# pvjosue/CWFA

Measured on AMD Instinct MI355X. Metric: volumes/sec inverse-pass @512×512×96 fp32; NLL match vs ref (1/2/4/8 GPU), higher is better.
Workload: dtype f32 (storage, accumulation, wavelets, couplings); convolution products on the bf16 matrix cores from an exact three-way bf16 split of both fp32 operands, six products per fp32 product: fp32-equivalent; plain-fp32-MFMA figure: fp32_mfma; 1 GPU; 512x512x96 volume, 4-scale CWFA (CAT blocks, 64 ch) + LRNN inverse, z=0, batch 1/GPU, random-init weights (BASELINE.json configs[2]); precision=split, parallelism=replicated x1 (independent volumes per GPU, no collective)

## Files before the change

### cwfa_amd/_lib.py

```python
import ctypes as C
import os

_HERE = os.path.dirname(os.path.abspath(__file__))
LIB_PATH = os.path.join(_HERE, "libcwfa_hip.so")

CLAMP = {"NONE": 0, "ATAN": 1, "TANH": 2, "SIGMOID": 3}
ACT = {None: 0, "none": 0, "elu": 1, "prelu": 2, "gelu": 3, "relu": 4}
CHAIN_MAX = 8

c_f32p = C.c_void_p
c_i64p = C.c_void_p
c_f64p = C.c_void_p


class AffineStage(C.Structure):
    _fields_ = [("s_raw", c_f32p), ("t", c_f32p), ("s_bs", C.c_int64), ("t_bs", C.c_int64), ("clamp_kind", C.c_int),
                ("clamp", C.c_float), ("pre_scale", C.c_float), ("t_neg_div_sqrt2", C.c_int), ("perm", c_i64p),
                ("perm_axis", C.c_int), ("gin", C.c_int)]


class Chain(C.Structure):
    _fields_ = [("n_stages", C.c_int), ("stage", AffineStage * CHAIN_MAX), ("src_c", C.c_void_p), ("src_h", C.c_void_p)]


class ChainGrads(C.Structure):
    _fields_ = [("ds", c_f32p * CHAIN_MAX), ("dt", c_f32p * CHAIN_MAX), ("ds_bs", C.c_int64 * CHAIN_MAX),
                ("dt_bs", C.c_int64 * CHAIN_MAX)]


class ConvOpts(C.Structure):
    _fields_ = [("bias", c_f32p), ("act", C.c_int), ("prelu_alpha", c_f32p), ("residual", c_f32p), ("res_bs", C.c_int64),
                ("act2", C.c_int), ("in_scale", c_f32p), ("in_shift", c_f32p), ("in_affine_bs", C.c_int), ("in_add", c_f32p),
                ("in_add_bs", C.c_int64), ("upshuffle2", C.c_int), ("in_blocked8", C.c_int), ("out_blocked8", C.c_int),
                ("in_cat", c_f32p), ("in_cat_bs", C.c_int64), ("in_cat_from", C.c_int), ("in_cat_c1", C.c_int), ("out_stats", c_f64p), ("prelu_per_channel", C.c_int)]


class Couple(C.Structure):
    _fields_ = [("x", c_f32p), ("y", c_f32p), ("x_bs", C.c_int64), ("y_bs", C.c_int64), ("n", C.c_int), ("clamp_kind", C.c_int),
                ("clamp", C.c_float), ("pre_scale", C.c_float), ("rev", C.c_int), ("logdet", c_f64p), ("in_blocked8", C.c_int)]


class EvalAffine(C.Structure):
    _fields_ = [("enabled", C.c_int), ("scale", C.c_float), ("std", C.c_float), ("mean", C.c_float)]


class EvalPost(C.Structure):
    _fields_ = [("normalize", C.c_int), ("threshold", C.c_int), ("norm_sub", C.c_float), ("norm_div", C.c_float),
                ("vol_min", C.c_float), ("lower", C.c_float), ("upper", C.c_float), ("clamp_value", C.c_float)]

# ... 12 lines not shown
    "cwfa_set_option": (i, [C.c_char_p, i]),
    "cwfa_haar1d_fwd_f32": (i, [p, p, p, i, i, i64, i64, i64, i64, p]),
    "cwfa_haar1d_inv_f32": (i, [p, p, p, i, i, i64, i64, i64, i64, p]),
    "cwfa_haar2d_fwd_f32": (i, [p, p, i, i, i, i, i, f, p]),
    "cwfa_haar2d_inv_f32": (i, [p, p, i, i, i, i, i, f, p]),
    "cwfa_haar3d_fwd_f32": (i, [p, p, i, i, i, i, i, f, i64, p]),
    "cwfa_haar3d_inv_f32": (i, [p, p, i, i, i, i, i, f, i64, p]),
    "cwfa_gather_f32": (i, [p, p, p, i, i, i, i, i, i64, i64, p]),
    "cwfa_affine_f32": (i, [p, p, C.POINTER(AffineStage), i, i, i, i, i, i64, i64, p, p, p]),
    "cwfa_channel_affine_f32": (i, [p, p, p, p, i, p, p, i, i, i64, i64, i64, p]),
    "cwfa_chain_inv_f32": (i, [p, p, p, C.POINTER(Chain), i, i, i, i, i64, i64, i64, p, p]),
    "cwfa_chain_fwd_f32": (i, [p, p, p, C.POINTER(Chain), p, i, i, i, i, i64, i64, i64, p, p, p]),
    "cwfa_conv2d_packed_floats": (i64, [i, i, i]),
    "cwfa_conv2d_pack_f32": (i, [p, p, i, i, i, i, p]),
    "cwfa_conv2d_f32": (i, [p, p, p, i, i, i, i, i, i, i64, i64, C.POINTER(ConvOpts), p]),
    "cwfa_subnet_pack1x1_f32": (i, [p, p, p]),
    "cwfa_subnet_layer_tape_f32": (i, [p, p, p, p, p, p, p, i, i, i, i64, i64, i64, p]),
    "cwfa_subnet_layer_f32": (i, [p, p, p, p, p, p, i, i, i, i64, i64, p]),
    "cwfa_conv3d_1k1_f32": (i, [p, p, p, p, p, p, p, i, i, i, i, i, p]),
    "cwfa_conv3d_1k1_split_f32": (i, [p, p, p, p, p, p, p, i, i, i, i, i, p]),
    "cwfa_channel_stats_f32": (i, [p, p, i, i, i64, i64, p]),
    "cwfa_bn_fold_f32": (i, [p, d, p, p, p, p, f, p, i, p, p, i, p]),
    "cwfa_maxpool_f32": (i, [p, p, p, p, p, i, i, i, i, i, i, p]),
    "cwfa_sample_stats_f32": (i, [p, p, i, i64, p]),
    "cwfa_layernorm_apply_f32": (i, [p, p, p, p, f, p, i, i64, p]),
    "cwfa_attention_combine_f32": (i, [p, p, p, p, p, p, p, p, i, i, i64, p]),
    "cwfa_scale_channels_f32": (i, [p, p, p, i, i, i64, p]),
    "cwfa_axpby_f32": (i, [p, p, f, f, p, i64, p]),
    "cwfa_bn_running_update_f32": (i, [p, C.c_double, f, p, p, p, i, p]),
    "cwfa_bn_finish_f32": (i, [p, d, p, p, p, f, i, p, p, f, p, p, f, f, i, p, p, i, i, p]),
# ... 87 lines not shown
```

### cwfa_amd/csrc/conv2d.hip

```cpp
#include "conv_internal.h"

#include <string.h>
#include <type_traits>

namespace {

template <int KS_, int CK_, int MT_, int NT_, int WM_, int WN_, int XV_ = 1>
struct Cfg {
    static constexpr int KS = KS_, CK = CK_, MT = MT_, NT = NT_, WM = WM_, WN = WN_;
    static constexpr int XV = XV_;
    static_assert(XV_ == 1 || (XV_ == 4 && KS_ == 1), "vector staging needs halo-free tiles");
    static constexpr int PAD = KS / 2;
    static constexpr int NTHREADS = 64 * WM * WN;
    static constexpr int CT = 32 * MT * WM;
    static constexpr int TR = NT * WN;
    static constexpr int TC = 32;
    static constexpr int XR = TR + KS - 1;
    static constexpr int XC = TC + KS - 1;
    static constexpr int XS = CK * XR * XC;
    static constexpr int XS_PAD = (XS + 3) & ~3;
    static constexpr int WS = KS * KS * CK * CT;
    static constexpr int XPT = (XS / XV + NTHREADS - 1) / NTHREADS;
    static constexpr int WPT = (WS / 4 + NTHREADS - 1) / NTHREADS;
    static constexpr int BUF = XS_PAD + WS;
// ... 557 lines not shown
namespace {

int fill_params(ConvParams& p, const char* name, const float* x, const float* w_packed, float* y, int B, int Cin, int H,
                int W, int Cout, int64_t x_bs, int64_t y_bs, const cwfa_conv_opts* opts) {
    CWFA_REQUIRE(B >= 0 && Cin > 0 && Cout > 0 && H >= 0 && W >= 0, CWFA_E_INVAL, "%s: bad size", name);
    if (B == 0 || H == 0 || W == 0) return 1;
    CWFA_REQUIRE(x && w_packed && y, CWFA_E_INVAL, "%s: null pointer", name);
    CWFA_REQUIRE((int64_t)Cin * H * W < (1ll << 30) && (int64_t)Cout * H * W * (p.o.upshuffle2 ? 1 : 1) < (1ll << 30), CWFA_E_SHAPE, "%s: C*H*W exceeds the 32-bit byte offsets of a tile (2^30 elements per image)", name);
    CWFA_REQUIRE(cwfa_aligned16(w_packed), CWFA_E_ALIGN, "%s: packed weights must be 16-byte aligned", name);
    p.x = x; p.wp = w_packed; p.y = y;
    p.B = B; p.Cin = Cin; p.H = H; p.W = W; p.Cout = Cout;
    p.x_bs = x_bs; p.y_bs = y_bs;
    p.products = g_cwfa_operand == CwfaOperand::split3 ? 6 : 1;
    if (opts) p.o = *opts;
    CWFA_REQUIRE(!(p.o.in_scale && !p.o.in_shift), CWFA_E_INVAL, "%s: in_scale without in_shift", name);
    CWFA_REQUIRE(p.o.act >= 0 && p.o.act <= CWFA_ACT_RELU && p.o.act2 >= 0 && p.o.act2 <= CWFA_ACT_RELU, CWFA_E_INVAL,
                 "%s: bad activation", name);
    CWFA_REQUIRE(!((p.o.act == CWFA_ACT_PRELU || p.o.act2 == CWFA_ACT_PRELU) && !p.o.prelu_alpha), CWFA_E_INVAL,
                 "%s: PReLU without prelu_alpha", name);
    return CWFA_OK;
}

typedef Cfg<1, 16, 2, 4, 4, 2> CS;
constexpr int CS_XB = 3 * 2 * 8 * 32 * 16, CS_WB = 3 * 2 * 256 * 16, CS_BUFB = CS_XB + CS_WB;

__device__ __forceinline__ void split3(float v, unsigned short (&o)[3]) {
    const __bf16 a1 = (__bf16)v;
    const float r1 = v - (float)a1;
    const __bf16 a2 = (__bf16)r1;
    const float r2 = r1 - (float)a2;
// ... 390 lines not shown
            default: return launch<C1v_128, N | U | K, U>(p, epi, st);
        }
    }
    switch (s.id) {
        case 0: return launch<C3_32, N | P | RP, 0>(p, epi, st);
        case 1: return launch<C3_64, N | E | P | RP, 0>(p, epi, st);
        case 2: return launch<C3_128, N | P, P>(p, epi, st);
        case 3: return launch<C1_32, N | P | G, P>(p, epi, st);
        case 4: return launch<C1_64, N | RE | G | K, 0>(p, epi, st);
        case 5: return launch<C1_128, N | U | K, U>(p, epi, st);
        case 6: return launch<C7_32, N, 0>(p, epi, st);
        default: return launch<C7_64, N, 0>(p, epi, st);
    }
}

extern "C" int cwfa_subnet_pack1x1_f32(const float* w, float* panel, void* stream) {
    CWFA_REQUIRE(w && panel, CWFA_E_INVAL, "cwfa_subnet_pack1x1_f32: null pointer");
    hipLaunchKernelGGL(pack1x1_kernel, dim3(16), dim3(256), 0, (hipStream_t)stream, w, panel);
    CWFA_LAUNCH_CHECK("cwfa_subnet_pack1x1_f32");
    return CWFA_OK;
}

extern "C" int cwfa_subnet_layer_tape_f32(const float* x, const float* w3_packed, const float* b3, const float* w1_panel,
                                          const float* b1, float* y, float* hidden, int B, int H, int W, int64_t x_bs, int64_t y_bs,
                                          int64_t hidden_bs, void* stream) {
    ConvParams p{};
    cwfa_conv_opts o{};
    o.bias = b3;
    int rc = fill_params(p, "cwfa_subnet_layer_tape_f32", x, w3_packed, y, B, 64, H, W, 64, x_bs, y_bs, &o);
    if (rc) return rc < 0 ? rc : CWFA_OK;
// ... 31 lines not shown
```

### cwfa_amd/csrc/conv_split3x3.hip

```cpp
#include "conv_internal.h"

extern int g_cwfa_split_xcd_map;
extern int g_cwfa_split_rows16;

namespace {

constexpr int TR = 8, TC = 32;

template <int KS, int RPW = 4>
struct XG {
    static constexpr int TRW = 2 * RPW, NT = 2 * RPW;
    static constexpr int PAD = KS / 2, XR = TRW + 2 * PAD, XC = TC + 2 * PAD, NTAP = KS * KS;
    static constexpr int EPK = XR * XC;
    static constexpr int KHB = KS == 7 ? 8512 : RPW == 8 ? 9792 : 5440;
    static constexpr int XPB = 2 * KHB;
    static constexpr int XB = 3 * XPB;
    static constexpr bool SPECIAL = KS == 3 && RPW == 4;
    static constexpr int NEK = SPECIAL ? 2 : 3;
    static_assert(EPK * 16 <= KHB && KHB % 256 == 64 && 2 * EPK <= 512 * NEK, "staging entry map");
    static_assert(!SPECIAL || (EPK > 256 && EPK <= 384), "3x3 staging entry map");
    static_assert(KS == 3 || RPW == 4, "7x7: 8-row tiles");
};

template <int MPW, int KS = 3, int RPW = 4, int WM = 4>
// ... 67 lines not shown
            ekh[k] = e >= EPK;
            eidx[k] = e - ekh[k] * EPK;
            fin[k] = e < 2 * EPK;
        }
    }
    bool fok[NEK];
#pragma unroll
    for (int k = 0; k < NEK; ++k) {
        const int r = eidx[k] / XC, c = eidx[k] % XC;
        const int gr = row0 + r - PAD, gc = col0 + c - PAD;
        fok[k] = fin[k] && gr >= 0 && gr < p.H && gc >= 0 && gc < p.W;
        fo[k] = !fok[k] ? OOB : p.o.in_blocked8 ? (unsigned)((gr * p.W + gc) * 32) : (unsigned)((gr * p.W + gc) * 4);
        if constexpr (!SPECIAL) fo[k] = !fok[k] ? OOB : fo[k] + (unsigned)(ekh[k] * 8) * (unsigned)plane;
    }
    const int xbytes = p.Cin * plane;
    const auto rx = CWFA_RSRC(p.x + (int64_t)b * p.x_bs, xbytes);
    const auto ra = CWFA_RSRC(ADD ? p.o.in_add + (int64_t)b * p.o.in_add_bs : p.x, ADD ? xbytes : 0);
    const bool has_aff = p.o.in_scale != nullptr;
    typedef const float __attribute__((address_space(4))) cfloat;
    cfloat* sc = has_aff ? (cfloat*)(p.o.in_scale + (int64_t)b * p.o.in_affine_bs) : nullptr;
    cfloat* sh = has_aff ? (cfloat*)(p.o.in_shift + (int64_t)b * p.o.in_affine_bs) : nullptr;

    auto load_entry = [&](auto kc, float (&xv)[8], float (&av)[8], int chunk) {
        constexpr int k = decltype(kc)::value;
        const int ch0 = chunk * 16 + (SPECIAL ? ekh[k] * 8 : 0);
        if (KS == 3 && !ADD && p.o.in_blocked8) {
            const f32x4 lo4 = __builtin_bit_cast(f32x4, __builtin_amdgcn_raw_buffer_load_b128(rx, fo[k], ch0 * plane, 0));
            const f32x4 hi4 = __builtin_bit_cast(f32x4, __builtin_amdgcn_raw_buffer_load_b128(rx, fo[k], ch0 * plane + 16, 0));
#pragma unroll
            for (int j = 0; j < 4; ++j) {
                xv[j] = lo4[j];
                xv[4 + j] = hi4[j];
// ... 515 lines not shown
    CWFA_REQUIRE(B >= 0 && Cin > 0 && Cout > 0 && H >= 0 && W >= 0, CWFA_E_INVAL, "cwfa_conv3x3_split_f32: bad size");
    if (B == 0 || H == 0 || W == 0) return CWFA_OK;
    CWFA_REQUIRE(x && w_packed && y, CWFA_E_INVAL, "cwfa_conv3x3_split_f32: null pointer");
    CWFA_REQUIRE(cwfa_aligned16(w_packed), CWFA_E_ALIGN, "cwfa_conv3x3_split_f32: packed weights must be 16-byte aligned");
    SParams p{};
    p.x = x; p.wp = w_packed; p.y = y;
    p.B = B; p.Cin = Cin; p.H = H; p.W = W; p.Cout = Cout; p.x_bs = x_bs; p.y_bs = y_bs;
    if (opts) p.o = *opts;
    CWFA_REQUIRE(!p.o.upshuffle2 && !p.o.in_cat, CWFA_E_SHAPE, "cwfa_conv3x3_split_f32: upshuffle2 / in_cat are 1x1 features");
    CWFA_REQUIRE(!p.o.in_blocked8 || (Cin % 8 == 0 && cwfa_aligned16(x) && (x_bs & 3) == 0 && !p.o.in_add), CWFA_E_ALIGN,
                 "cwfa_conv3x3_split_f32: blocked input needs Cin %% 8 == 0, 16-byte alignment and no added tensor");
    CWFA_REQUIRE(!p.o.out_blocked8 || (Cout % 8 == 0 && cwfa_aligned16(y) && (y_bs & 3) == 0 && !p.o.residual && p.o.act2 == CWFA_ACT_NONE &&
                                       (p.o.act == CWFA_ACT_NONE || p.o.act == CWFA_ACT_PRELU)),
                 CWFA_E_ALIGN, "cwfa_conv3x3_split_f32: blocked output needs Cout %% 8 == 0, 16-byte alignment and a bias / PReLU epilogue");
    CWFA_REQUIRE(!(p.o.in_scale && !p.o.in_shift), CWFA_E_INVAL, "cwfa_conv3x3_split_f32: in_scale without in_shift");
    CWFA_REQUIRE(!p.o.out_stats || (!p.o.out_blocked8 && !p.o.residual && p.o.act2 == CWFA_ACT_NONE &&
                                    (p.o.act == CWFA_ACT_NONE || p.o.act == CWFA_ACT_PRELU)),
                 CWFA_E_INVAL, "cwfa_conv3x3_split_f32: out_stats needs an NCHW output and a bias / PReLU epilogue");
    CWFA_REQUIRE(!((p.o.out_stats || p.o.out_blocked8) && p.o.in_add && p.o.act == CWFA_ACT_NONE), CWFA_E_INVAL,
                 "cwfa_conv3x3_split_f32: out_stats / out_blocked8 with in_add need a PReLU epilogue");
    CWFA_REQUIRE(p.o.act >= 0 && p.o.act <= CWFA_ACT_RELU && p.o.act2 >= 0 && p.o.act2 <= CWFA_ACT_RELU, CWFA_E_INVAL,
                 "cwfa_conv3x3_split_f32: bad activation");
    CWFA_REQUIRE(!((p.o.act == CWFA_ACT_PRELU || p.o.act2 == CWFA_ACT_PRELU) && !p.o.prelu_alpha), CWFA_E_INVAL,
                 "cwfa_conv3x3_split_f32: PReLU without prelu_alpha");
    p.nchunks = (Cin + 15) / 16;
    p.nsteps = nsteps_of(Cin);
    p.nrun = p.nsteps - ((p.nchunks & 1) ? 4 : 0);
    p.tiles_x = (W + TC - 1) / TC;
    const int mpw = mpw_of(Cout);
    CWFA_REQUIRE((int64_t)(Cin + 64) * H * W * 4 < (1ll << 31) && (int64_t)(Cout + 64 * mpw) * H * W * 4 < (1ll << 31) &&
// ... 40 lines not shown
    pack_bank(w, packed, Cout, Cin, 64, 49, (hipStream_t)stream);
    CWFA_LAUNCH_CHECK("cwfa_conv7x7_split_pack_f32");
    return CWFA_OK;
}

extern "C" int cwfa_conv7x7_split_f32(const float* x, const void* w_packed, float* y, int B, int Cin, int H, int W, int Cout,
                                      int64_t x_bs, int64_t y_bs, const cwfa_conv_opts* opts, void* stream) {
    CWFA_REQUIRE(B >= 0 && Cin > 0 && Cout > 0 && Cout <= 64 && H >= 0 && W >= 0, CWFA_E_INVAL, "cwfa_conv7x7_split_f32: bad size (Cout <= 64)");
    if (B == 0 || H == 0 || W == 0) return CWFA_OK;
    CWFA_REQUIRE(x && w_packed && y, CWFA_E_INVAL, "cwfa_conv7x7_split_f32: null pointer");
    CWFA_REQUIRE(cwfa_aligned16(w_packed), CWFA_E_ALIGN, "cwfa_conv7x7_split_f32: packed weights must be 16-byte aligned");
    SParams p{};
    p.x = x; p.wp = w_packed; p.y = y;
    p.B = B; p.Cin = Cin; p.H = H; p.W = W; p.Cout = Cout; p.x_bs = x_bs; p.y_bs = y_bs;
    if (opts) p.o = *opts;
    CWFA_REQUIRE(!p.o.upshuffle2 && !p.o.in_cat && !p.o.in_scale && !p.o.in_add && !p.o.in_blocked8 && !p.o.out_blocked8 && !p.o.residual && !p.o.out_stats &&
                     p.o.act == CWFA_ACT_NONE && p.o.act2 == CWFA_ACT_NONE,
                 CWFA_E_INVAL, "cwfa_conv7x7_split_f32: bias-only epilogue, no load-side prologue, NCHW maps");
    p.nchunks = (Cin + 15) / 16;
    p.nsteps = nsteps_of(Cin, 49);
    p.nrun = p.nsteps;
    p.tiles_x = (W + TC - 1) / TC;
    CWFA_REQUIRE((int64_t)(Cin + 64) * H * W * 4 < (1ll << 31) && (int64_t)(Cout + 64) * H * W * 4 < (1ll << 31), CWFA_E_SHAPE,
                 "cwfa_conv7x7_split_f32: one sample's input / output must stay below 2 GiB");
    CWFA_REQUIRE((int64_t)p.tiles_x * ((H + TR - 1) / TR) < (1ll << 31) && B <= 65535, CWFA_E_SHAPE, "cwfa_conv7x7_split_f32: grid too large");
    hipStream_t st = (hipStream_t)stream;
    return launch<2, false, CWFA_ACT_NONE, 7, 4, 2>(p, st);
}
```

### cwfa_amd/ops.py

```python
import ctypes as C

import torch

from . import _lib
from ._lib import AffineStage, Chain, ConvOpts, check

__all__ = ["haar1d", "haar2d", "gather", "affine", "channel_affine", "chain_inv", "chain_fwd", "pack_conv_weight",
           "conv2d", "conv2d_wgrad", "elu_bwd", "set_precision", "gelu_add", "gelu_bwd", "layernorm_bwd", "attention_bwd", "plane_affine", "bn_bwd_stats", "bn_act_bwd", "maxpool2_bwd", "chain_bwd", "chain_inv_bwd", "prelu_bwd", "conv3d_1k1_backward", "pack_1x1_panel", "pack_split_layer_weight", "subnet_layer", "conv3d_1k1", "channel_stats", "bn_fold", "bn_running_update", "maxpool", "sample_stats", "layernorm_apply",
           "attention_combine", "scale_channels", "axpby", "stage"]


def _stream():
    return C.c_void_p(torch.cuda.current_stream().cuda_stream)


def _p(t):
    return None if t is None else C.c_void_p(t.data_ptr())


def _dev(t, name="tensor"):
    if not torch.is_tensor(t):
        raise TypeError(f"{name}: expected a torch.Tensor, got {type(t)}")
    if not t.is_cuda:
        raise RuntimeError(f"{name}: cwfa_amd runs on MI355X only -- got a {t.device} tensor (no CPU fallback exists)")
# ... 361 lines not shown
    start = (c1 + 15) // 16 * 16
    wz = torch.zeros((cout, start + cin - c1, 1, 1), dtype=torch.float32, device=w.device)
    wz[:, :c1] = w[:, :c1]
    wz[:, start:] = w[:, c1:]
    pc = pack_conv_weight(wz)
    pc.version, pc.src_ptr = w._version, w.data_ptr()
    pc.cat_c1, pc.cat_from = c1, start
    return pc


def conv_writes_stats(pc, act=None, residual=None, act2=None, out_blocked=False, in_add=False):
    return bool(pc.split and pc.ks == 3 and act in (None, "prelu") and residual is None and act2 is None and not out_blocked
                and not (in_add and act is None))


def conv2d(x, pc, bias=None, act=None, prelu_alpha=None, residual=None, act2=None, in_scale=None, in_shift=None,
           in_add=None, out=None, in_blocked=False, out_blocked=False, cat=None, out_stats=None):
    L = _lib.lib()
    x, xbs = planes(x, "x")
    B, Cin, H, W = x.shape
    o = ConvOpts()
    keep = [x]
    if cat is not None:
        cat, cbs = planes(cat, "cat")
        c1 = getattr(pc, "cat_c1", None)
        if c1 is None or Cin != c1 or tuple(cat.shape) != (B, pc.cin - pc.cat_from, H, W) or in_scale is not None or in_add is not None:
            raise ValueError("conv2d: `cat` needs a bank from pack_conv_weight_cat for exactly these two inputs, and no load-side prologue")
        o.in_cat, o.in_cat_bs, o.in_cat_from, o.in_cat_c1 = cat.data_ptr(), cbs, pc.cat_from, c1
        keep.append(cat)
        Cin = pc.cin
    if Cin != pc.cin:
        raise ValueError(f"conv2d: input has {Cin} channels, filter bank expects {pc.cin}")
# ... 26 lines not shown
            raise ValueError(f"conv2d: residual {tuple(residual.shape)} != output {oshape}")
        o.residual, o.res_bs = residual.data_ptr(), rbs
        keep.append(residual)
    if in_scale is not None:
        o.in_scale, o.in_shift = _dev(in_scale).data_ptr(), _dev(in_shift).data_ptr()
        if in_scale.numel() not in (Cin, B * Cin) or in_shift.numel() != in_scale.numel():
            raise ValueError("conv2d: in_scale / in_shift must be [Cin] or [B,Cin]")
        o.in_affine_bs = Cin if (in_scale.numel() == B * Cin and B > 1) else 0
    if in_add is not None:
        in_add, abs_ = planes(in_add, "in_add")
        if tuple(in_add.shape) != tuple(x.shape):
            raise ValueError("conv2d: in_add shape mismatch")
        o.in_add, o.in_add_bs = in_add.data_ptr(), abs_
        keep.append(in_add)
    o.upshuffle2 = int(up)
    if in_blocked:
        if not (pc.split and pc.ks == 3):
            raise ValueError("conv2d: channel-blocked input is read by the split-bf16 3x3 kernel only")
        o.in_blocked8 = 1
    if out_blocked:
        ok3 = (pc.split and pc.ks == 3 and pc.cout % 8 == 0 and residual is None and act2 is None and act in (None, "prelu")
               and not split3x3_narrow(pc.cout) and not (in_add is not None and act is None))
        ok1 = not pc.split and pc.ks == 1 and pc.cout >= 33 and pc.cout % 8 == 0 and not up
        if not (ok3 or ok1):
            raise ValueError("conv2d: channel-blocked output is written by the split-bf16 3x3 kernel (bias / PReLU) and by the "
                             "direct 1x1 kernel with 40..64 output channels only")
        o.out_blocked8 = 1
    if out_stats is not None:
        if not conv_writes_stats(pc, act, residual, act2, out_blocked, in_add is not None):
            raise ValueError("conv2d: out_stats needs the split-bf16 3x3 kernel with an NCHW output and a bias / PReLU epilogue")
# ... 27 lines not shown
                                       for i in range(B)], 0)
                if in_add is not None:
                    x = axpby(x.contiguous(), 1.0, in_add, 1.0)
            x, xbs = planes(x, "x")
            o.in_scale = o.in_shift = o.in_add = None
        check(L.cwfa_conv3x3_split_f32(_p(x), _p(pc.packed), _p(out), B, Cin, H, W, pc.cout, xbs, ybs, C.byref(o),
                                       _stream()), "conv3x3_split")
    elif pc.split:
        ws = torch.empty(L.cwfa_split_workspace_bytes(B, Cin, H * W), dtype=torch.uint8, device=x.device)
        per_sample = in_scale is not None and in_scale.numel() == B * Cin and B > 1
        check(L.cwfa_split_input_f32(_p(x), _p(ws), B, Cin, H * W, xbs, _p(in_scale), _p(in_shift), Cin if per_sample else 0,
                                     _p(in_add), in_add.stride(0) if in_add is not None else 0, _stream()), "split_input")
        o.in_scale = o.in_shift = o.in_add = None
        check(L.cwfa_conv_split_f32(_p(ws), _p(pc.packed), _p(out), B, Cin, H, W, pc.cout, pc.ks, ybs, C.byref(o), _stream()),
              "conv_split")
    else:
        check(L.cwfa_conv2d_f32(_p(x), _p(pc.packed), _p(out), B, Cin, H, W, pc.cout, pc.ks, xbs, ybs, C.byref(o),
                                _stream()), "conv2d")
    if rec is not None and rec.want(key):
        e1.record()
        rec.add(key, e0, e1)
    return out


def pack_couple_weight(w, bias):
    L = _lib.lib()
    w = _dev(w, "weight").detach()
    n2, cin, ks, kw = w.shape
    if ks != 3 or kw != 3 or n2 % 2 or n2 // 2 > 64:
        raise ValueError(f"pack_couple_weight: a [2n,Cin,3,3] bank with n <= 64 is needed, got {tuple(w.shape)}")
# ... 923 lines not shown
```

### cwfa_amd/unet.py

```python
import torch
from torch import nn

from . import ops
from .amp import amp_entry

__all__ = ["UNet", "UNetConvBlock", "UNetUpBlock"]


_MATERIALIZE_UP = False
_MATERIALIZE = True


class _Packed:

    def __init__(self):
        self._c = {}

    def get(self, conv, transposed=False):
        w = conv.weight
        pc = self._c.get(id(conv))
        if pc is None or pc.version != w._version or pc.src_ptr != w.data_ptr() or pc.epoch != ops.pack_epoch():
            pc = self._c[id(conv)] = ops.pack_conv_weight(w, transposed=transposed)
        return pc


class _Drop:
    __slots__ = ("u", "p")

    def __init__(self, u, p):
        self.u, self.p = u, p

    def mask(self):
        return ((self.u >= self.p).to(torch.float32) / (1.0 - self.p)).contiguous()


STATS_IN_EPILOGUE = True


def _bn_batch_stats(bn):
    return bn.training or not bn.track_running_stats


def _bn_stats_buffer(bn, device):
    key = (str(device), torch.cuda.current_stream(device).cuda_stream)
    bufs = bn.__dict__.setdefault("_cwfa_stats", {})
    st = bufs.get(key)
    if st is None or getattr(bn, "_cwfa_stats_dirty", False):
        st = bufs[key] = torch.zeros(2 * bn.num_features, dtype=torch.float64, device=device)
    bn._cwfa_stats_dirty = True
    return st

# ... 72 lines not shown
        step = 3 if self.batch_norm else 2
        return [(mods[i], mods[i + 1], mods[i + 2] if self.batch_norm else None) for i in (0, step)]

    @staticmethod
    def _act(a):
        if isinstance(a, nn.PReLU):
            if a.weight.numel() != 1:
                raise NotImplementedError("per-channel PReLU")
            return "prelu", a.weight
        if isinstance(a, nn.ELU):
            return "elu", None
        if isinstance(a, nn.ReLU):
            return "relu", None
        raise NotImplementedError(f"activation {type(a).__name__} has no HIP epilogue")

    def run(self, x, in_affine=None, in_add=None, out_mask=None):
        aff = in_affine
        layers = self._layers()
        packs = [self._packed.get(conv) for conv, _, _ in layers]
        for li, (conv, act, bn) in enumerate(layers):
            kind, alpha = self._act(act)
            sc, sh = aff if aff is not None else (None, None)
            add = in_add if li == 0 else None
            if (_MATERIALIZE and ops._split_bf16 < 2 and (sc is not None or add is not None)
                    and (x.shape[2] * x.shape[3]) % 4 == 0):
                x = ops.plane_affine(x, sc, sh, add=add)
                sc = sh = add = None
            st = None
            if (STATS_IN_EPILOGUE and bn is not None and _bn_batch_stats(bn)
                    and ops.conv_writes_stats(packs[li], kind, in_add=add is not None)):
                st = _bn_stats_buffer(bn, x.device)
            x = ops.conv2d(x, packs[li], bias=conv.bias, act=kind, prelu_alpha=alpha, in_scale=sc,
                           in_shift=sh, in_add=add, out_stats=st)
            last = li == len(layers) - 1
            m = out_mask if last else None
            if bn is not None:
                aff = _bn_affine(bn, x, m, stats=st)
            elif m is not None:
                aff = _drop_affine(x.shape[1], m)
            else:
                aff = None
        return x, aff

    @amp_entry
    def forward(self, x):
        y, aff = self.run(x)
        if aff is None:
            return y
# ... 7 lines not shown
        super().__init__()
        self.skip_conn = skip_conn
        if up_mode != 'upconv':
            raise NotImplementedError("cwfa_amd UNetUpBlock: up_mode='upconv' only (what the LRNN uses, networks.py:532)")
        self.up = nn.ConvTranspose2d(in_size, out_size, kernel_size=2, stride=2, bias=use_bias)
        in_size = out_size if not skip_conn else in_size // 2
        self.conv_block = UNetConvBlock(in_size, out_size, padding, batch_norm, use_bias=use_bias, activation=activation)
        self._packed = _Packed()

    @staticmethod
    def center_crop(layer, target_size):
        _, _, h, w = layer.size()
        dy, dx = (h - target_size[0]) // 2, (w - target_size[1]) // 2
        return layer[:, :, dy:(dy + target_size[0]), dx:(dx + target_size[1])]

    def run(self, x, bridge, in_affine=None, out_mask=None):
        sc, sh = in_affine if in_affine is not None else (None, None)
        if _MATERIALIZE_UP and ops._split_bf16 < 1 and sc is not None and (x.shape[2] * x.shape[3]) % 4 == 0:
            x = ops.plane_affine(x, sc, sh)
            sc = sh = None
        up = ops.conv2d(x, self._packed.get(self.up, transposed=True), bias=self.up.bias, in_scale=sc, in_shift=sh)
        add = self.center_crop(bridge, up.shape[2:]) if self.skip_conn else None
        return self.conv_block.run(up, in_add=add, out_mask=out_mask)

    @amp_entry
    def forward(self, x, bridge):
        y, aff = self.run(x, bridge)
        return y if aff is None else ops.channel_affine(y, aff[0], aff[1])


class UNet(nn.Module):

    def __init__(self, in_channels=1, n_classes=2, depth=5, wf=6, padding=True, batch_norm=True, up_mode='upsample',
                 drop_out=0, use_bias=False, skip_conn=False, activation=nn.PReLU):
        super().__init__()
        assert up_mode in ('upconv', 'upsample')
        self.padding, self.depth, self.skip_conn, self.drop_out = padding, depth, skip_conn, drop_out
        prev = in_channels
# ... 13 lines not shown
    @amp_entry
    def forward(self, x, store_activations=False, in_affine=None):
        if store_activations:
            raise NotImplementedError("store_activations is a debugging aid of the reference, not on the hot path")
        B, dev = x.shape[0], x.device
        skips, aff = [], in_affine
        n_draw = 0
        if self.drop_out:
            n_draw = B * (sum(d.block[0].out_channels for d in list(self.down_path)[:-1]) +
                          sum(u.conv_block.block[0].out_channels for u in self.up_path))
        pool = _DrawPool(n_draw, dev)
        for i, down in enumerate(self.down_path):
            x, aff = down.run(x, in_affine=aff)
            if i != len(self.down_path) - 1:
                sc, sh = aff if aff is not None else (None, None)
                x, full = ops.maxpool(x, x.shape[-1] // 2, x.shape[-1] // 2, sc, sh, want_full=True)
                skips.append(full)
                m = _drop(self.drop_out, B, x.shape[1], dev, pool)
                aff = _drop_affine(x.shape[1], m) if m is not None else None
        for i, up in enumerate(self.up_path):
            m = _drop(self.drop_out, B, up.conv_block.block[0].out_channels, dev, pool)
            x, aff = up.run(x, skips[-i - 1], in_affine=aff, out_mask=m)
        kind, alpha = UNetConvBlock._act(self.last[1])
        sc, sh = aff if aff is not None else (None, None)
        return ops.conv2d(x, self._packed.get(self.last[0]), bias=self.last[0].bias, act=kind, prelu_alpha=alpha,
                          in_scale=sc, in_shift=sh)
```

### include/cwfa_hip.h

```cpp
#ifndef CWFA_HIP_H
#define CWFA_HIP_H

#include <stdint.h>

#ifdef __cplusplus
extern "C" {
#endif

#define CWFA_VERSION 100

enum {
    CWFA_OK = 0,
    CWFA_E_INVAL = -1,
    CWFA_E_SHAPE = -2,
    CWFA_E_ALIGN = -3,
    CWFA_E_HIP = -4
};

enum { CWFA_CLAMP_NONE = 0, CWFA_CLAMP_ATAN = 1, CWFA_CLAMP_TANH = 2, CWFA_CLAMP_SIGMOID = 3 };

enum { CWFA_ACT_NONE = 0, CWFA_ACT_ELU = 1, CWFA_ACT_PRELU = 2, CWFA_ACT_GELU = 3, CWFA_ACT_RELU = 4 };

int cwfa_version(void);
const char* cwfa_last_error(void);
// ... 69 lines not shown
    int64_t res_bs;
    int act2;
    const float* in_scale;
    const float* in_shift;
    int in_affine_bs;
    const float* in_add;
    int64_t in_add_bs;
    int upshuffle2;
    int in_blocked8;
    int out_blocked8;
    const float* in_cat;
    int64_t in_cat_bs;
    int in_cat_from, in_cat_c1;
    double* out_stats;
    int prelu_per_channel;
} cwfa_conv_opts;

int cwfa_conv2d_f32(const float* x, const float* w_packed, float* y, int B, int Cin, int H, int W, int Cout, int ks,
                    int64_t x_bs, int64_t y_bs, const cwfa_conv_opts* opts, void* stream);

int cwfa_subnet_pack1x1_f32(const float* w, float* panel, void* stream);
int cwfa_subnet_layer_f32(const float* x, const float* w3_packed, const float* b3, const float* w1_panel, const float* b1,
                          float* y, int B, int H, int W, int64_t x_bs, int64_t y_bs, void* stream);
int cwfa_subnet_layer_tape_f32(const float* x, const float* w3_packed, const float* b3, const float* w1_panel, const float* b1,
                               float* y, float* hidden, int B, int H, int W, int64_t x_bs, int64_t y_bs, int64_t hidden_bs,
                               void* stream);

int cwfa_conv3d_1k1_f32(const float* x, const float* w1, const float* b1, const float* alpha, const float* w2,
                        const float* b2, float* y, int B, int D, int H, int W, int K, void* stream);
int cwfa_conv3d_1k1_split_f32(const float* x, const float* w1, const float* b1, const float* alpha, const float* w2,
                              const float* b2, float* y, int B, int D, int H, int W, int K, void* stream);


int cwfa_channel_stats_f32(const float* x, double* stats, int B, int C, int64_t HW, int64_t x_bs, void* stream);
// ... 161 lines not shown
```

Baseline: 53.95 volumes/s.

## Fuse skip-affine into up-path conv and add streaming narrow 1x1 conv kernel

Down-path skips are now kept raw (pre-BN-affine) together with their scale/shift. The first up-path split 3x3 conv applies that affine on the in_add operand, by swapping the roles of the x and add buffers. This avoids writing the full-resolution affined skip tensor during maxpool. A separate streaming kernel handles 1x1 convs with at most 8 outputs and 64 to 1024 inputs: it splits channels across four waves, keeps weights and the affine in LDS, and reduces partial sums in LDS. That kernel runs in plain fp32 FMA rather than the split path, and the fused-affine path is limited to certain output-bank widths.

After: 54.10 volumes/s (median of 6 runs). Within noise of the previous version (+0.3%).

```diff
diff --git a/cwfa_amd/_lib.py b/cwfa_amd/_lib.py
--- a/cwfa_amd/_lib.py
+++ b/cwfa_amd/_lib.py
@@ -32,7 +32,8 @@
     _fields_ = [("bias", c_f32p), ("act", C.c_int), ("prelu_alpha", c_f32p), ("residual", c_f32p), ("res_bs", C.c_int64),
                 ("act2", C.c_int), ("in_scale", c_f32p), ("in_shift", c_f32p), ("in_affine_bs", C.c_int), ("in_add", c_f32p),
                 ("in_add_bs", C.c_int64), ("upshuffle2", C.c_int), ("in_blocked8", C.c_int), ("out_blocked8", C.c_int),
-                ("in_cat", c_f32p), ("in_cat_bs", C.c_int64), ("in_cat_from", C.c_int), ("in_cat_c1", C.c_int), ("out_stats", c_f64p), ("prelu_per_channel", C.c_int)]
+                ("in_cat", c_f32p), ("in_cat_bs", C.c_int64), ("in_cat_from", C.c_int), ("in_cat_c1", C.c_int), ("out_stats", c_f64p), ("prelu_per_channel", C.c_int),
+                ("in_affine_on_add", C.c_int)]
 
 
 class Couple(C.Structure):
@@ -75,6 +76,7 @@
     "cwfa_conv2d_packed_floats": (i64, [i, i, i]),
     "cwfa_conv2d_pack_f32": (i, [p, p, i, i, i, i, p]),
     "cwfa_conv2d_f32": (i, [p, p, p, i, i, i, i, i, i, i64, i64, C.POINTER(ConvOpts), p]),
+    "cwfa_conv1x1_stream_f32": (i, [p, p, p, i, i, i64, i, i64, i64, C.POINTER(ConvOpts), p]),
     "cwfa_subnet_pack1x1_f32": (i, [p, p, p]),
     "cwfa_subnet_layer_tape_f32": (i, [p, p, p, p, p, p, p, i, i, i, i64, i64, i64, p]),
     "cwfa_subnet_layer_f32": (i, [p, p, p, p, p, p, i, i, i, i64, i64, p]),
diff --git a/cwfa_amd/csrc/conv2d.hip b/cwfa_amd/csrc/conv2d.hip
--- a/cwfa_amd/csrc/conv2d.hip
+++ b/cwfa_amd/csrc/conv2d.hip
@@ -595,6 +595,7 @@
     p.products = g_cwfa_operand == CwfaOperand::split3 ? 6 : 1;
     if (opts) p.o = *opts;
     CWFA_REQUIRE(!(p.o.in_scale && !p.o.in_shift), CWFA_E_INVAL, "%s: in_scale without in_shift", name);
+    CWFA_REQUIRE(!p.o.in_affine_on_add, CWFA_E_INVAL, "%s: in_affine_on_add is a cwfa_conv3x3_split_f32 feature", name);
     CWFA_REQUIRE(p.o.act >= 0 && p.o.act <= CWFA_ACT_RELU && p.o.act2 >= 0 && p.o.act2 <= CWFA_ACT_RELU, CWFA_E_INVAL,
                  "%s: bad activation", name);
     CWFA_REQUIRE(!((p.o.act == CWFA_ACT_PRELU || p.o.act2 == CWFA_ACT_PRELU) && !p.o.prelu_alpha), CWFA_E_INVAL,
@@ -1015,6 +1016,109 @@
     }
 }
 
+constexpr int S1_KG = 4, S1_ENT = 12, S1_MAXC = 1024;
+
+template <int CO>
+__global__ __launch_bounds__(64 * S1_KG) void conv1x1_stream_kernel(const float* __restrict__ x, const float* __restrict__ wp,
+                                                                    float* __restrict__ y, int Cin, int64_t HW, int64_t x_bs, int64_t y_bs,
+                                                                    cwfa_conv_opts o) {
+    extern __shared__ __attribute__((aligned(16))) float smem[];
+    const int tid = threadIdx.x, lane = tid & 63;
+    const int kg = __builtin_amdgcn_readfirstlane(tid >> 6);
+    const int b = blockIdx.y;
+    const bool aff = o.in_scale != nullptr;
+    for (int i = tid; i < Cin * S1_ENT; i += 64 * S1_KG) {
+        const int c = i / S1_ENT, j = i % S1_ENT;
+        float v = 0.f;
+        if (j < CO) v = wp[c * C1_32::CT + j];
+        else if (j == 8) v = aff ? o.in_scale[(int64_t)b * o.in_affine_bs + c] : 1.f;
+        else if (j == 9) v = aff ? o.in_shift[(int64_t)b * o.in_affine_bs + c] : 0.f;
+        smem[i] = v;
+    }
+    __syncthreads();
+    const int64_t q = (int64_t)blockIdx.x * 64 + lane, nq = HW >> 2;
+    const bool ok = q < nq;
+    const float* xp = x + (int64_t)b * x_bs + 4 * (ok ? q : 0);
+    const int cq = (Cin + S1_KG - 1) / S1_KG, c0 = kg * cq, c1 = c0 + cq < Cin ? c0 + cq : Cin;
+    f32x4 acc[CO];
+#pragma unroll
+    for (int k = 0; k < CO; ++k) acc[k] = f32x4{0.f, 0.f, 0.f, 0.f};
+    auto mac = [&](f32x4 v, int c) {
+        const f32x4* e = reinterpret_cast<const f32x4*>(smem + c * S1_ENT);
+        const f32x4 w0 = e[0], w1 = CO > 4 ? e[1] : f32x4{0.f, 0.f, 0.f, 0.f}, a = e[2];
+        if (aff) v = v * a[0] + a[1];
+#pragma unroll
+        for (int k = 0; k < CO; ++k) {
+            const float w = k < 4 ? w0[k & 3] : w1[k & 3];
+#pragma unroll
+            for (int i = 0; i < 4; ++i) acc[k][i] = __builtin_fmaf(w, v[i], acc[k][i]);
+        }
+    };
+    constexpr int U = 8;
+    int c = c0;
+    for (; c + U <= c1; c += U) {
+        f32x4 v[U];
+#pragma unroll
+        for (int u = 0; u < U; ++u) v[u] = *reinterpret_cast<const f32x4*>(xp + (int64_t)(c + u) * HW);
+#pragma unroll
+        for (int u = 0; u < U; ++u) mac(v[u], c + u);
+    }
+    for (; c < c1; ++c) mac(*reinterpret_cast<const f32x4*>(xp + (int64_t)c * HW), c);
+    __syncthreads();
+    f32x4* red = reinterpret_cast<f32x4*>(smem);
+    if (kg > 0) {
+#pragma unroll
+        for (int k = 0; k < CO; ++k) red[((kg - 1) * CO + k) * 64 + lane] = acc[k];
+    }
+    __syncthreads();
+    if (kg != 0 || !ok) return;
+    const float alpha = o.act == CWFA_ACT_PRELU ? *o.prelu_alpha : 0.f;
+    float* yp = y + (int64_t)b * y_bs + 4 * q;
+#pragma unroll
+    for (int k = 0; k < CO; ++k) {
+        f32x4 v = acc[k];
+#pragma unroll
+        for (int g = 0; g < S1_KG - 1; ++g) v = v + red[(g * CO + k) * 64 + lane];
+        const float bias = o.bias ? o.bias[k] : 0.f;
+#pragma unroll
+        for (int i = 0; i < 4; ++i) v[i] = cwfa_act(v[i] + bias, o.act, alpha);
+        *reinterpret_cast<f32x4*>(yp + (int64_t)k * HW) = v;
+    }
+}
+
+extern "C" int cwfa_conv1x1_stream_f32(const float* x, const float* w_packed, float* y, int B, int Cin, int64_t HW, int Cout,
+                                       int64_t x_bs, int64_t y_bs, const cwfa_conv_opts* opts, void* stream) {
+    CWFA_REQUIRE(B >= 0 && Cin > 0 && Cout > 0 && HW >= 0, CWFA_E_INVAL, "cwfa_conv1x1_stream_f32: bad size");
+    CWFA_REQUIRE(Cout <= 8 && Cin <= S1_MAXC && (HW & 3) == 0 && B <= 65535 && HW / 256 < (1ll << 31), CWFA_E_SHAPE,
+                 "cwfa_conv1x1_stream_f32: needs Cout <= 8, Cin <= %d, HW %% 4 == 0", S1_MAXC);
+    if (B == 0 || HW == 0) return CWFA_OK;
+    CWFA_REQUIRE(x && w_packed && y, CWFA_E_INVAL, "cwfa_conv1x1_stream_f32: null pointer");
+    CWFA_REQUIRE(cwfa_aligned16(x) && cwfa_aligned16(y) && (x_bs & 3) == 0 && (y_bs & 3) == 0, CWFA_E_ALIGN,
+                 "cwfa_conv1x1_stream_f32: x / y must be 16-byte aligned with batch strides that are multiples of 4");
+    cwfa_conv_opts o{};
+    if (opts) o = *opts;
+    CWFA_REQUIRE(!o.residual && o.act2 == CWFA_ACT_NONE && !o.in_add && !o.upshuffle2 && !o.in_blocked8 && !o.out_blocked8 && !o.in_cat &&
+                     !o.out_stats && !o.prelu_per_channel && !o.in_affine_on_add && (o.act == CWFA_ACT_NONE || o.act == CWFA_ACT_PRELU),
+                 CWFA_E_INVAL, "cwfa_conv1x1_stream_f32: bias, act = NONE | PRELU and in_scale / in_shift only");
+    CWFA_REQUIRE(!o.in_scale == !o.in_shift, CWFA_E_INVAL, "cwfa_conv1x1_stream_f32: in_scale and in_shift go together");
+    CWFA_REQUIRE(o.act != CWFA_ACT_PRELU || o.prelu_alpha, CWFA_E_INVAL, "cwfa_conv1x1_stream_f32: PReLU without prelu_alpha");
+    const dim3 grid((unsigned)((HW / 4 + 63) / 64), B);
+    const int table = Cin * S1_ENT * 4, sums = (S1_KG - 1) * Cout * 64 * 16;
+    const int lds = table > sums ? table : sums;
+#define CWFA_S1(CO)                                                                                                              \
+    case CO:                                                                                                                     \
+        hipLaunchKernelGGL(conv1x1_stream_kernel<CO>, grid, dim3(64 * S1_KG), lds, (hipStream_t)stream, x, w_packed, y, Cin, HW, \
+                           x_bs, y_bs, o);                                                                                       \
+        break
+    switch (Cout) {
+        CWFA_S1(1); CWFA_S1(2); CWFA_S1(3); CWFA_S1(4); CWFA_S1(5); CWFA_S1(6); CWFA_S1(7);
+        default: CWFA_S1(8);
+    }
+#undef CWFA_S1
+    CWFA_LAUNCH_CHECK("cwfa_conv1x1_stream_f32");
+    return CWFA_OK;
+}
+
 extern "C" int cwfa_subnet_pack1x1_f32(const float* w, float* panel, void* stream) {
     CWFA_REQUIRE(w && panel, CWFA_E_INVAL, "cwfa_subnet_pack1x1_f32: null pointer");
     hipLaunchKernelGGL(pack1x1_kernel, dim3(16), dim3(256), 0, (hipStream_t)stream, w, panel);
diff --git a/cwfa_amd/csrc/conv_split3x3.hip b/cwfa_amd/csrc/conv_split3x3.hip
--- a/cwfa_amd/csrc/conv_split3x3.hip
+++ b/cwfa_amd/csrc/conv_split3x3.hip
@@ -105,8 +105,10 @@
         if constexpr (!SPECIAL) fo[k] = !fok[k] ? OOB : fo[k] + (unsigned)(ekh[k] * 8) * (unsigned)plane;
     }
     const int xbytes = p.Cin * plane;
-    const auto rx = CWFA_RSRC(p.x + (int64_t)b * p.x_bs, xbytes);
-    const auto ra = CWFA_RSRC(ADD ? p.o.in_add + (int64_t)b * p.o.in_add_bs : p.x, ADD ? xbytes : 0);
+    const bool swap = ADD && p.o.in_affine_on_add != 0;
+    const float* xa = ADD ? p.o.in_add + (int64_t)b * p.o.in_add_bs : p.x;
+    const auto rx = CWFA_RSRC(swap ? xa : p.x + (int64_t)b * p.x_bs, xbytes);
+    const auto ra = CWFA_RSRC(swap ? p.x + (int64_t)b * p.x_bs : xa, ADD ? xbytes : 0);
     const bool has_aff = p.o.in_scale != nullptr;
     typedef const float __attribute__((address_space(4))) cfloat;
     cfloat* sc = has_aff ? (cfloat*)(p.o.in_scale + (int64_t)b * p.o.in_affine_bs) : nullptr;
@@ -652,6 +654,8 @@
                                        (p.o.act == CWFA_ACT_NONE || p.o.act == CWFA_ACT_PRELU)),
                  CWFA_E_ALIGN, "cwfa_conv3x3_split_f32: blocked output needs Cout %% 8 == 0, 16-byte alignment and a bias / PReLU epilogue");
     CWFA_REQUIRE(!(p.o.in_scale && !p.o.in_shift), CWFA_E_INVAL, "cwfa_conv3x3_split_f32: in_scale without in_shift");
+    CWFA_REQUIRE(!p.o.in_affine_on_add || (p.o.in_scale && p.o.in_add && wm_of(Cout) == 4), CWFA_E_INVAL,
+                 "cwfa_conv3x3_split_f32: in_affine_on_add needs in_scale / in_shift, in_add and a bank with 49 .. 64 or > 96 outputs");
     CWFA_REQUIRE(!p.o.out_stats || (!p.o.out_blocked8 && !p.o.residual && p.o.act2 == CWFA_ACT_NONE &&
                                     (p.o.act == CWFA_ACT_NONE || p.o.act == CWFA_ACT_PRELU)),
                  CWFA_E_INVAL, "cwfa_conv3x3_split_f32: out_stats needs an NCHW output and a bias / PReLU epilogue");
@@ -722,7 +726,7 @@
     p.x = x; p.wp = w_packed; p.y = y;
     p.B = B; p.Cin = Cin; p.H = H; p.W = W; p.Cout = Cout; p.x_bs = x_bs; p.y_bs = y_bs;
     if (opts) p.o = *opts;
-    CWFA_REQUIRE(!p.o.upshuffle2 && !p.o.in_cat && !p.o.in_scale && !p.o.in_add && !p.o.in_blocked8 && !p.o.out_blocked8 && !p.o.residual && !p.o.out_stats &&
+    CWFA_REQUIRE(!p.o.upshuffle2 && !p.o.in_cat && !p.o.in_scale && !p.o.in_add && !p.o.in_affine_on_add && !p.o.in_blocked8 && !p.o.out_blocked8 && !p.o.residual && !p.o.out_stats &&
                      p.o.act == CWFA_ACT_NONE && p.o.act2 == CWFA_ACT_NONE,
                  CWFA_E_INVAL, "cwfa_conv7x7_split_f32: bias-only epilogue, no load-side prologue, NCHW maps");
     p.nchunks = (Cin + 15) / 16;
diff --git a/cwfa_amd/ops.py b/cwfa_amd/ops.py
--- a/cwfa_amd/ops.py
+++ b/cwfa_amd/ops.py
@@ -399,8 +399,16 @@
                 and not (in_add and act is None))
 
 
+STREAM_1X1 = True
+STREAM_1X1_MIN_CIN = 64
+
+
+def conv_takes_add_affine(pc):
+    return bool(pc.split and pc.ks == 3 and not split3x3_narrow(pc.cout))
+
+
 def conv2d(x, pc, bias=None, act=None, prelu_alpha=None, residual=None, act2=None, in_scale=None, in_shift=None,
-           in_add=None, out=None, in_blocked=False, out_blocked=False, cat=None, out_stats=None):
+           in_add=None, out=None, in_blocked=False, out_blocked=False, cat=None, out_stats=None, in_affine_on_add=False):
     L = _lib.lib()
     x, xbs = planes(x, "x")
     B, Cin, H, W = x.shape
@@ -457,6 +465,11 @@
         o.in_add, o.in_add_bs = in_add.data_ptr(), abs_
         keep.append(in_add)
     o.upshuffle2 = int(up)
+    if in_affine_on_add:
+        if in_scale is None or in_add is None or not conv_takes_add_affine(pc):
+            raise ValueError("conv2d: in_affine_on_add needs in_scale / in_shift, in_add and a bank of the split-bf16 3x3 kernel with "
+                             "49 .. 64 or more than 96 outputs")
+        o.in_affine_on_add = 1
     if in_blocked:
         if not (pc.split and pc.ks == 3):
             raise ValueError("conv2d: channel-blocked input is read by the split-bf16 3x3 kernel only")
@@ -514,6 +527,11 @@
         o.in_scale = o.in_shift = o.in_add = None
         check(L.cwfa_conv_split_f32(_p(ws), _p(pc.packed), _p(out), B, Cin, H, W, pc.cout, pc.ks, ybs, C.byref(o), _stream()),
               "conv_split")
+    elif (STREAM_1X1 and pc.ks == 1 and not up and pc.cout <= 8 and STREAM_1X1_MIN_CIN <= Cin <= 1024 and (H * W) % 4 == 0
+          and residual is None and act2 is None and act in (None, "prelu") and in_add is None and cat is None and not out_blocked
+          and x.data_ptr() % 16 == 0 and out.data_ptr() % 16 == 0 and xbs % 4 == 0 and ybs % 4 == 0):
+        check(L.cwfa_conv1x1_stream_f32(_p(x), _p(pc.packed), _p(out), B, Cin, H * W, pc.cout, xbs, ybs, C.byref(o), _stream()),
+              "conv1x1_stream")
     else:
         check(L.cwfa_conv2d_f32(_p(x), _p(pc.packed), _p(out), B, Cin, H, W, pc.cout, pc.ks, xbs, ybs, C.byref(o),
                                 _stream()), "conv2d")
diff --git a/cwfa_amd/unet.py b/cwfa_amd/unet.py
--- a/cwfa_amd/unet.py
+++ b/cwfa_amd/unet.py
@@ -35,6 +35,7 @@
 
 
 STATS_IN_EPILOGUE = True
+RAW_SKIPS = True
 
 
 def _bn_batch_stats(bn):
@@ -137,15 +138,23 @@
             return "relu", None
         raise NotImplementedError(f"activation {type(a).__name__} has no HIP epilogue")
 
-    def run(self, x, in_affine=None, in_add=None, out_mask=None):
+    def takes_raw_skip(self):
+        return ops.conv_takes_add_affine(self._packed.get(self._layers()[0][0]))
+
+    def run(self, x, in_affine=None, in_add=None, out_mask=None, add_affine=None):
         aff = in_affine
         layers = self._layers()
         packs = [self._packed.get(conv) for conv, _, _ in layers]
+        if add_affine is not None and (in_affine is not None or in_add is None):
+            raise ValueError("UNetConvBlock.run: add_affine goes with in_add and without in_affine")
         for li, (conv, act, bn) in enumerate(layers):
             kind, alpha = self._act(act)
             sc, sh = aff if aff is not None else (None, None)
             add = in_add if li == 0 else None
-            if (_MATERIALIZE and ops._split_bf16 < 2 and (sc is not None or add is not None)
+            on_add = li == 0 and add_affine is not None
+            if on_add:
+                sc, sh = add_affine
+            if (_MATERIALIZE and ops._split_bf16 < 2 and (sc is not None or add is not None) and not on_add
                     and (x.shape[2] * x.shape[3]) % 4 == 0):
                 x = ops.plane_affine(x, sc, sh, add=add)
                 sc = sh = add = None
@@ -154,7 +163,7 @@
                     and ops.conv_writes_stats(packs[li], kind, in_add=add is not None)):
                 st = _bn_stats_buffer(bn, x.device)
             x = ops.conv2d(x, packs[li], bias=conv.bias, act=kind, prelu_alpha=alpha, in_scale=sc,
-                           in_shift=sh, in_add=add, out_stats=st)
+                           in_shift=sh, in_add=add, out_stats=st, in_affine_on_add=on_add)
             last = li == len(layers) - 1
             m = out_mask if last else None
             if bn is not None:
@@ -192,14 +201,14 @@
         dy, dx = (h - target_size[0]) // 2, (w - target_size[1]) // 2
         return layer[:, :, dy:(dy + target_size[0]), dx:(dx + target_size[1])]
 
-    def run(self, x, bridge, in_affine=None, out_mask=None):
+    def run(self, x, bridge, in_affine=None, out_mask=None, bridge_affine=None):
         sc, sh = in_affine if in_affine is not None else (None, None)
         if _MATERIALIZE_UP and ops._split_bf16 < 1 and sc is not None and (x.shape[2] * x.shape[3]) % 4 == 0:
             x = ops.plane_affine(x, sc, sh)
             sc = sh = None
         up = ops.conv2d(x, self._packed.get(self.up, transposed=True), bias=self.up.bias, in_scale=sc, in_shift=sh)
         add = self.center_crop(bridge, up.shape[2:]) if self.skip_conn else None
-        return self.conv_block.run(up, in_add=add, out_mask=out_mask)
+        return self.conv_block.run(up, in_add=add, out_mask=out_mask, add_affine=bridge_affine if self.skip_conn else None)
 
     @amp_entry
     def forward(self, x, bridge):
@@ -243,13 +252,22 @@
             x, aff = down.run(x, in_affine=aff)
             if i != len(self.down_path) - 1:
                 sc, sh = aff if aff is not None else (None, None)
-                x, full = ops.maxpool(x, x.shape[-1] // 2, x.shape[-1] // 2, sc, sh, want_full=True)
-                skips.append(full)
+                half = x.shape[-1] // 2
+                raw = (RAW_SKIPS and self.skip_conn and sc is not None and ops._split_bf16 >= 2
+                       and x.shape[2] == 2 * half and x.shape[3] == 2 * half
+                       and self.up_path[len(self.down_path) - 2 - i].conv_block.takes_raw_skip())
+                if raw:
+                    skips.append((x, (sc, sh)))
+                    x = ops.maxpool(x, half, half, sc, sh)
+                else:
+                    x, full = ops.maxpool(x, half, half, sc, sh, want_full=True)
+                    skips.append((full, None))
                 m = _drop(self.drop_out, B, x.shape[1], dev, pool)
                 aff = _drop_affine(x.shape[1], m) if m is not None else None
         for i, up in enumerate(self.up_path):
             m = _drop(self.drop_out, B, up.conv_block.block[0].out_channels, dev, pool)
-            x, aff = up.run(x, skips[-i - 1], in_affine=aff, out_mask=m)
+            bridge, baff = skips[-i - 1]
+            x, aff = up.run(x, bridge, in_affine=aff, out_mask=m, bridge_affine=baff)
         kind, alpha = UNetConvBlock._act(self.last[1])
         sc, sh = aff if aff is not None else (None, None)
         return ops.conv2d(x, self._packed.get(self.last[0]), bias=self.last[0].bias, act=kind, prelu_alpha=alpha,
diff --git a/include/cwfa_hip.h b/include/cwfa_hip.h
--- a/include/cwfa_hip.h
+++ b/include/cwfa_hip.h
@@ -107,10 +107,13 @@
     int in_cat_from, in_cat_c1;
     double* out_stats;
     int prelu_per_channel;
+    int in_affine_on_add;
 } cwfa_conv_opts;
 
 int cwfa_conv2d_f32(const float* x, const float* w_packed, float* y, int B, int Cin, int H, int W, int Cout, int ks,
                     int64_t x_bs, int64_t y_bs, const cwfa_conv_opts* opts, void* stream);
+int cwfa_conv1x1_stream_f32(const float* x, const float* w_packed, float* y, int B, int Cin, int64_t HW, int Cout, int64_t x_bs,
+                            int64_t y_bs, const cwfa_conv_opts* opts, void* stream);
 
 int cwfa_subnet_pack1x1_f32(const float* w, float* panel, void* stream);
 int cwfa_subnet_layer_f32(const float* x, const float* w3_packed, const float* b3, const float* w1_panel, const float* b1,
```
